# mx-mark/VideoTransformer-pytorch

Measured on AMD Instinct MI355X. Metric: clips/sec TimeSformer-B divided_space_time 8x3x224x224 fwd+bwd (whole job), higher is better.
Workload: dtype bf16

## Files before the change

### videotransformer-pytorch_amd/csrc/api.hip

```cpp
#include <limits.h>
#include <stdarg.h>
#include <stdlib.h>
#include <string.h>
#include <string>
#include <vector>
#include "common.h"

namespace vtx {

static thread_local char g_err[512] = "";

void set_error(const char* fmt, ...) {
  va_list ap;
  va_start(ap, fmt);
  vsnprintf(g_err, sizeof(g_err), fmt, ap);
  va_end(ap);
}

int check_launch(const char* what) {
  hipError_t e = hipGetLastError();
  if (e != hipSuccess) {
    set_error("%s: launch failed: %s", what, hipGetErrorString(e));
    return VTX_ELAUNCH;
  }
  return VTX_OK;
}

static const char* const kNtNames[] = {"auto", "pp256", "dma2", "ring128x3", "ring128x4k32", "ring256x3", "ring256x3k32", "ring256x4k32"};
static const char* const kAttnF32Names[] = {"valu", "mfma"};
static const char* const kTnNames[] = {"auto", "pp256", "ring", "dma2", "w4"};

enum OptKind { OPT_FLAG, OPT_INT, OPT_CLAMP, OPT_ENUM, OPT_ADDR };
struct OptRow { const char* id[2]; OptKind kind; int Options::*field; int lo, hi, mult; const char* const* names; };
#define VTX_ENUM(names) 0, (int)(sizeof(names) / sizeof(*names)) - 1, 1, names
static const OptRow kOptions[] = {
    {{"VTX_GEMM_NT", "gemm_nt"}, OPT_ENUM, &Options::gemm_nt, VTX_ENUM(kNtNames)},
    {{"VTX_GEMM_TN", "gemm_tn"}, OPT_ENUM, &Options::gemm_tn, VTX_ENUM(kTnNames)},
    {{"VTX_GEMM_NODMA", "gemm_nodma"}, OPT_FLAG, &Options::gemm_nodma},
    {{"VTX_TN_SAFE", "tn_safe"}, OPT_FLAG, &Options::tn_safe},
    {{"VTX_TN_CUS", "tn_cus"}, OPT_INT, &Options::tn_cus, 32, 1024, 1},
    {{"VTX_ATTN_VALU", "attn_valu"}, OPT_FLAG, &Options::attn_valu},
    {{"VTX_ATTN_LONG", "attn_long"}, OPT_FLAG, &Options::attn_long},
    {{"VTX_ATTN_F32", "attn_f32"}, OPT_ENUM, &Options::attn_f32, VTX_ENUM(kAttnF32Names)},
    {{"VTX_ATTN_HD", "attn_hd"}, OPT_ENUM, &Options::attn_hd, VTX_ENUM(kAttnF32Names)},
    {{"VTX_ATTN_HW_FWD", "attn_hw_fwd"}, OPT_INT, &Options::attn_hw_fwd, 0, INT_MAX, 1},
    {{"VTX_ATTN_HW_BWD", "attn_hw_bwd"}, OPT_INT, &Options::attn_hw_bwd, 0, INT_MAX, 1},
    {{"VTX_ATTN_FUSED", "attn_fused"}, OPT_CLAMP, &Options::attn_fused, 0, 2},
    {{"VTX_ATTN_FWD_STREAM", "attn_fwd_stream"}, OPT_FLAG, &Options::attn_fwd_stream},
    {{"VTX_ATTN_DKV", "attn_dkv"}, OPT_INT, &Options::attn_dkv, 0, 4, 1},
    {{"VTX_GEMM_PP_GRID", "pp_grid"}, OPT_INT, &Options::pp_grid, 8, 4096, 8},
    {{"VTX_GEMM_PP_CG", "pp_cg"}, OPT_INT, &Options::pp_cg, 0, INT_MAX, 1},
    {{"VTX_GEMM_PP_EPI", "pp_epi"}, OPT_INT, &Options::pp_epi, INT_MIN, INT_MAX, 1},
    {{"VTX_GEMM_PP_CONT", "pp_cont"}, OPT_FLAG, &Options::pp_cont},
// ... 161 lines not shown
```

### videotransformer-pytorch_amd/csrc/common.h

```cpp
#pragma once
#include <hip/hip_runtime.h>
#include <stdint.h>
#include <atomic>
#include <stdio.h>
#include "../../include/vtx.h"

namespace vtx {

typedef __attribute__((ext_vector_type(8))) __bf16 bf16x8;
typedef __attribute__((ext_vector_type(4))) __bf16 bf16x4;
typedef __attribute__((ext_vector_type(4))) float f32x4;
typedef __attribute__((ext_vector_type(4))) unsigned int u32x4;
typedef __attribute__((ext_vector_type(16))) float f32x16;
typedef __attribute__((ext_vector_type(4))) short s16x4;
typedef unsigned short bf16raw;

__host__ __device__ inline float bf2f(bf16raw v) {
  union { uint32_t u; float f; } c; c.u = ((uint32_t)v) << 16; return c.f;
}
__host__ __device__ inline bf16raw f2bf(float f) {
#if defined(__HIP_DEVICE_COMPILE__)
  union { __bf16 b; bf16raw r; } c; c.b = (__bf16)f; return c.r;
#else
  union { uint32_t u; float f; } c; c.f = f;
// ... 97 lines not shown
#pragma clang fp contract(off)
  float cdf, g;
  gelu_parts(x, cdf, g);
  return x * cdf;
}
__device__ inline float gelu_erf_grad(float x) {
#pragma clang fp contract(off)
  float cdf, g;
  gelu_parts(x, cdf, g);
  const float xs = x * 0.3989422804014327f;
  return fmaf(xs, g, cdf);
}
__device__ inline void gelu_erf_both(float x, float& val, float& grad) {
#pragma clang fp contract(off)
  float cdf, g;
  gelu_parts(x, cdf, g);
  const float xs = x * 0.3989422804014327f;
  grad = fmaf(xs, g, cdf);
  val = x * cdf;
}

enum { NT_AUTO = 0, NT_PP256, NT_DMA2, NT_RING128X3, NT_RING128X4K32, NT_RING256X3, NT_RING256X3K32, NT_RING256X4K32,
       NT_REG, NT_F32 };
enum { TN_AUTO = 0, TN_PP256, TN_RING, TN_DMA2, TN_W4 };
struct Options {
  int gemm_nt = NT_AUTO;
  int gemm_tn = TN_AUTO;
  int gemm_nodma = 0;
  int tn_safe = 0;
  int tn_cus = 256;
  int attn_valu = 0;
  int attn_long = 1;
  int attn_f32 = 1;
  int attn_hw_fwd = 16;
  int attn_hw_bwd = 4;
  int attn_fused = 2;
  int attn_fwd_stream = 1;
  int attn_dkv = 3;
  int ln_rows = 3;
  int pp_grid = 256;
  int pp_cg = 0;
  int pp_epi = 0;
  int pp_cont = 1;
  unsigned long long pp_trace = 0;
  int attn_hd = 1;
};
Options& options();
// ... 48 lines not shown
```

### videotransformer-pytorch_amd/csrc/gemm_tn.hip

```cpp
#include <stdlib.h>
#include <string>
#include "gemm_common.h"

namespace vtx {

struct TnOut {
  float* slab; long slab_stride;
  int N1, N2;
  float* cslab;
  int cs_fold;
};

struct TnTile { int split, t1, t2, r0, c0, m_begin, m_end; };
template <int TM, int TC, bool REMAINDER, typename Id>
__device__ __forceinline__ TnTile tn_tile_of(Id bid, int M, int m_per_split, int tiles2, int tiles12) {
  TnTile t;
  t.split = bid / tiles12;
  const int tile = bid - t.split * tiles12;
  t.t1 = tile / tiles2; t.t2 = tile - t.t1 * tiles2;
  t.r0 = t.t1 * TM; t.c0 = t.t2 * TC;
  t.m_begin = t.split * m_per_split;
  if (REMAINDER) t.m_end = (t.split == (int)(gridDim.x / tiles12) - 1) ? M : t.m_begin + m_per_split;
  else t.m_end = min(M, t.m_begin + m_per_split);
  return t;
}
template <int TM, int TC, bool REMAP, bool REMAINDER>
__device__ __forceinline__ TnTile tn_tile(int M, int m_per_split, int tiles2, int tiles12) {
  if (REMAP) return tn_tile_of<TM, TC, REMAINDER>(xcd_remap(blockIdx.x, gridDim.x), M, m_per_split, tiles2, tiles12);
  return tn_tile_of<TM, TC, REMAINDER>((unsigned)blockIdx.x, M, m_per_split, tiles2, tiles12);
}

template <int NI, int NJ>
__device__ __forceinline__ void tn_zero(f32x16 (&acc)[NI][NJ]) {
#pragma unroll
  for (int i = 0; i < NI; ++i)
#pragma unroll
    for (int j = 0; j < NJ; ++j)
#pragma unroll
      for (int r = 0; r < 16; ++r) acc[i][j][r] = 0.f;
}

__device__ __forceinline__ void tn_cs_add(float (&cs)[8], const u32x4& v) {
#pragma unroll
  for (int j = 0; j < 4; ++j) {
    cs[2 * j] += __uint_as_float(v[j] << 16);
    cs[2 * j + 1] += __uint_as_float(v[j] & 0xffff0000u);
  }
}
template <int TC, int NV>
__device__ __forceinline__ void tn_cs_put(float* red, int row_lane, int col, const float (&cs)[NV]) {
#pragma unroll
  for (int j = 0; j < NV; ++j) red[row_lane * TC + col + j] = cs[j];
}
template <int RL, int TC>
__device__ __forceinline__ void tn_cs_fold(const float* red, const TnOut& o, const TnTile& t, int copy, int tid) {
  __syncthreads();
  if (tid < TC && t.r0 + tid < o.N1) {
    float a = 0.f;
#pragma unroll
    for (int r = 0; r < RL; ++r) a += red[r * TC + tid];
    o.cslab[(long)t.split * o.slab_stride + (long)copy * o.N1 + t.r0 + tid] = a;
  }
  __syncthreads();
// ... 14 lines not shown
  }
}

template <int LD>
__device__ __forceinline__ bf16x8 tn_tr_pair(const bf16raw* p) {
  union { bf16x8 v; s16x4 h[2]; } u;
  u.h[0] = __builtin_amdgcn_ds_read_tr16_b64_v4i16((s16x4 __attribute__((address_space(3)))*)(p));
  u.h[1] = __builtin_amdgcn_ds_read_tr16_b64_v4i16((s16x4 __attribute__((address_space(3)))*)(p + 4 * LD));
  return u.v;
}
typedef __attribute__((address_space(3))) char tn_lds_char;
template <int OFF> __device__ inline s16x4 tn_tr_read(unsigned addr) {
  s16x4 d;
  asm volatile("ds_read_b64_tr_b16 %0, %1 offset:%2" : "=v"(d) : "v"(addr), "n"(OFF) : "memory");
  return d;
}
template <int OFF, int ROW4>
__device__ __forceinline__ bf16x8 tn_tr_frag(unsigned addr) {
  union { bf16x8 v; s16x4 h[2]; } u;
  u.h[0] = tn_tr_read<OFF>(addr);
  u.h[1] = tn_tr_read<OFF + ROW4>(addr);
  return u.v;
}

template <int ROWS, int CHUNKS, int THREADS>
__device__ __forceinline__ void tn_stage_ragged(bf16raw* dst, const bf16raw* __restrict__ src, long ld, const vtx_rowmap& map,
                                                int mt, int m_end, int col0, int ncols, int tid) {
  constexpr int RPP = THREADS / CHUNKS;
#pragma unroll
  for (int it = 0; it < ROWS / RPP; ++it) {
    const int row = tid / CHUNKS + RPP * it;
    const int lc = (tid % CHUNKS) ^ ((row & 3) << 2);
    uint4 v = make_uint4(0, 0, 0, 0);
    if (mt + row < m_end && col0 + lc * 8 < ncols)
      v = *reinterpret_cast<const uint4*>(src + map_row(map, mt + row) * ld + col0 + lc * 8);
    *reinterpret_cast<uint4*>(dst + row * (8 * CHUNKS) + (tid % CHUNKS) * 8) = v;
  }
}

constexpr int TN_BKM = 64;
constexpr int TN_LD = 160;
constexpr int TN_BKM32 = 16;
constexpr int TN_LD32 = 128;

template <bool SAFE>
__global__ __launch_bounds__(NT_THREADS) void gemm_tn_bf16_kernel(
// ... 389 lines not shown
    tn_cs_put<256>(red, cs_row, cs_chunk * 8, csum);
    tn_cs_fold<16, 256>(red, out, t, t2, tid);
  }
  float* stg = reinterpret_cast<float*>(smem) + wave * 32 * STAGE_LD;
#pragma unroll
  for (int mi = 0; mi < 2; ++mi) {
    stage_acc_half(stg, acc[mi], lane);
    __builtin_amdgcn_s_waitcnt(0xc07f);
    __builtin_amdgcn_wave_barrier();
    tn_store<4, STAGE_LD, 1>(out, stg, t.split, r0 + wm * 64 + mi * 32, c0 + wn * 64 + (lane & 7) * 8, lane);
    __builtin_amdgcn_s_waitcnt(0xc07f);
    __builtin_amdgcn_wave_barrier();
  }
}

constexpr int TP_BK = 64, TP_THREADS = 512;
constexpr int TP_REGION = TP_BK * 128;
constexpr int TP_BUF = 4 * TP_REGION;
constexpr int TP_RING_BYTES = 2 * TP_BUF * 2;
constexpr int TP_STG_LD = 64;
constexpr int TP_LDS_BYTES = TP_RING_BYTES + 8 * 16 * TP_STG_LD * 4;

constexpr int TP_FAR = 1 << 28;
template <int PPW>
struct TnFeeder {
  bf16raw* lds;
  int wave, lane, last_valid;
  long lda, ldb;
  int grp_a, grp_b;
  int prow0, rc, acol_l;
  unsigned voff_a, voff_b;
  int trm[4], crs[4], vld[4];
  const char* sp[4];
  long step64_a, step64_b;
  long skipb_a, skipb_b;

  __device__ __forceinline__ TnFeeder(bf16raw* lds_, int wave_, int lane_, const bf16raw* A, long lda_, const vtx_rowmap& amap,
                                      const bf16raw* B, long ldb_, const vtx_rowmap& bmap, int M, const TnTile& t, int last_valid_)
      : lds(lds_), wave(wave_), lane(lane_), last_valid(last_valid_), lda(lda_), ldb(ldb_), grp_a(amap.grp), grp_b(bmap.grp) {
    const int pc0 = wave * PPW, sub = pc0 >> 3;
    prow0 = (pc0 & 7) * 8 + (lane >> 3);
    rc = sub * 64 + ((lane & 7) ^ (((prow0 >> 1) & 1) << 2)) * 8;
    acol_l = (rc >> 6) * 128 + (rc & 63);
    voff_a = 2u * (unsigned)(prow0 * (int)lda + acol_l); voff_b = 2u * (unsigned)(prow0 * (int)ldb + rc);
    step64_a = 2L * TP_BK * lda; step64_b = 2L * TP_BK * ldb;
    skipb_a = 2L * amap.skip * lda; skipb_b = 2L * bmap.skip * ldb;
#pragma unroll
    for (int k = 0; k < 4; ++k) {
      const bool isA = k == 0 || k == 3;
      const vtx_rowmap& mp = isA ? amap : bmap;
      const int g = mp.grp;
      const int q = g > 0 ? t.m_begin / g : 0;
      trm[k] = g > 0 ? t.m_begin - q * g : 0;
      crs[k] = g > 0 ? g - trm[k] : TP_FAR;
      vld[k] = M - t.m_begin;
      const long phys0 = (long)mp.base + t.m_begin + (long)q * mp.skip;
      sp[k] = reinterpret_cast<const char*>(isA ? A + phys0 * lda + t.r0 + (k == 3 ? 64 : 0) : B + phys0 * ldb + t.c0 + (k == 2 ? 128 : 0));
    }
  }
  __device__ __forceinline__ bf16raw* piece(int kind, int kt, int j) const {
    return lds + (kt & 1) * TP_BUF + kind * TP_REGION + wave * (PPW * 512) + j * 512;
  }
  __device__ __forceinline__ void issue_piece(int kind, int kt, int j) {
    bf16raw* dst = piece(kind, kt, j);
    const bool isA = kind == 0 || kind == 3;
    const char* lo = sp[kind];
    const char* hi = lo + (isA ? skipb_a : skipb_b);
    const unsigned vo = isA ? voff_a : voff_b, vc = 2u * (unsigned)(isA ? acol_l : rc);
    const unsigned step8 = 16u * (unsigned)(isA ? lda : ldb);
    const int row = prow0 + 8 * j;
    if (crs[kind] >= TP_BK && vld[kind] >= TP_BK) {
      const unsigned m0v = (unsigned)(unsigned long)(tn_lds_char*)dst;
      asm volatile("s_mov_b32 m0, %2\n\ts_nop 0\n\tglobal_load_lds_dwordx4 %0, %1"
                   :: "v"(vo + j * step8), "s"(lo), "s"(m0v) : "memory", "m0");
      return;
    }
    const char* base = row >= crs[kind] ? hi : lo;
    const unsigned o = row < vld[kind] ? vo + j * step8 : vc;
    dma16(reinterpret_cast<const bf16raw*>(base + o), dst);
  }
  __device__ __forceinline__ void issue(int kind, int kt) {
#pragma unroll
    for (int j = 0; j < PPW; ++j) issue_piece(kind, kt, j);
  }
  __device__ __forceinline__ void advance(int kind) {
    const bool isA = kind == 0 || kind == 3;
    const int g = isA ? grp_a : grp_b;
    sp[kind] += isA ? step64_a : step64_b;
    vld[kind] -= TP_BK;
    if (g > 0) {
      trm[kind] += TP_BK;
      if (trm[kind] >= g) { trm[kind] -= g; sp[kind] += isA ? skipb_a : skipb_b; }
      crs[kind] = g - trm[kind];
    }
  }
  __device__ __forceinline__ void zero_tail(int kt) {
#pragma unroll
    for (int kind = 0; kind < 4; ++kind)
#pragma unroll
      for (int j = 0; j < PPW; ++j)
        if (prow0 + 8 * j >= last_valid) *reinterpret_cast<uint4*>(piece(kind, kt, j) + lane * 8) = make_uint4(0, 0, 0, 0);
  }
};

template <int R>
struct TnCsLane {
  unsigned sub, row, pc;
  __device__ __forceinline__ explicit TnCsLane(unsigned tid) : sub(tid / (8 * R)), row((tid >> 3) & (R - 1)), pc(tid & 7) {}
  __device__ __forceinline__ unsigned lds_off() const { return sub * 4096 + row * 64 + pc * 8; }
  __device__ __forceinline__ int tile_col() const { return sub * 128 + (pc ^ (((row >> 1) & 1) << 2)) * 8; }
};

template <int HALF>
__device__ __forceinline__ void tn_epi16(const TnOut& o, float* stg, const f32x16& a0, const f32x16& a1, int split, int r_base, int c, int lane) {
  const int col = lane & 31, rhalf = (lane >> 5) * 4;
#pragma unroll
  for (int r = 0; r < 8; ++r) stg[((r & 3) + 8 * (r >> 2) + rhalf) * TP_STG_LD + col] = a0[8 * HALF + r];
#pragma unroll
  for (int r = 0; r < 8; ++r) stg[((r & 3) + 8 * (r >> 2) + rhalf) * TP_STG_LD + 32 + col] = a1[8 * HALF + r];
  lgkm0();
  __builtin_amdgcn_wave_barrier();
  tn_store<2, TP_STG_LD, 2>(o, stg, split, r_base, c, lane);
  lgkm0();
  __builtin_amdgcn_wave_barrier();
}

template <bool TRACE>
__global__ __launch_bounds__(TP_THREADS, 2) void gemm_tn_bf16_pp_kernel(
    int M, int m_per_split, const bf16raw* __restrict__ A, long lda, vtx_rowmap amap,
    const bf16raw* __restrict__ B, long ldb, vtx_rowmap bmap, int tiles2, int tiles12, TnOut out, long long* __restrict__ trace) {
  extern __shared__ __attribute__((aligned(16))) char smem[];
  bf16raw* lds = reinterpret_cast<bf16raw*>(smem);
  const int tid = threadIdx.x, lane = tid & 63;
  const int wave = __builtin_amdgcn_readfirstlane(tid >> 6);
  const int wr = wave >> 2, wc = wave & 3;
  int trace_kt = -1;
  auto stamp = [&](int e) {
    if constexpr (TRACE) {
      if (tid == 0 && trace_kt >= 0)
        trace[((long)blockIdx.x * 8 + trace_kt) * 24 + e] = (long long)__builtin_amdgcn_s_memtime();
    }
  };
  const TnTile t = tn_tile<256, 256, true, true>(M, m_per_split, tiles2, tiles12);
  const int t2 = t.t2, r0 = t.r0, c0 = t.c0;
  const int span = t.m_end - t.m_begin;
  const int nk = (span + TP_BK - 1) / TP_BK;
  const int last_valid = span - (nk - 1) * TP_BK;
  TnFeeder<2> fd(lds, wave, lane, A, lda, amap, B, ldb, bmap, M, t, last_valid);

  f32x16 acc[4][2];
  tn_zero(acc);

  const int tr_row = 8 * (lane >> 5) + ((lane & 15) >> 2);
  const int tr_sw = ((lane >> 3) & 1) << 2;
  const int cl = 16 * ((lane >> 4) & 1) + 4 * (lane & 3);
  int fa_off[2], fb_off;
#pragma unroll
  for (int i = 0; i < 2; ++i) {
    const int cc = i * 32 + cl;
    fa_off[i] = wr * 4096 + tr_row * 64 + (((cc >> 3) ^ tr_sw) << 3) + (cc & 7);
  }
  {
    const int cc = (wc & 1) * 32 + cl;
    fb_off = (wc >> 1) * 4096 + tr_row * 64 + (((cc >> 3) ^ tr_sw) << 3) + (cc & 7);
  }
  const unsigned lds_b = (unsigned)(unsigned long)(tn_lds_char*)smem;
  const unsigned fa_addr[2] = {lds_b + 2u * fa_off[0], lds_b + 2u * fa_off[1]}, fb_addr = lds_b + 2u * fb_off;
  const bool want_cs = out.cslab != nullptr;
  bool do_cs = false;
  int cs_next = t2;
  float cs0[8] = {0, 0, 0, 0, 0, 0, 0, 0}, cs1[8] = {0, 0, 0, 0, 0, 0, 0, 0};
#define TP_COLSUM(buf_, kind_, cs_)                                                                      \
  if (do_cs) {                                                                                           \
    u32x4 v_[2];                                                                                         \
                                 \
    unsigned t_ = threadIdx.x;                                                                           \
    asm volatile("" : "+v"(t_));                                                                         \
    const unsigned ca_ = lds_b + 2u * ((t_ >> 8) * 4096 + ((t_ >> 3) & 31) * 64 + (t_ & 7) * 8);        \
    asm volatile("ds_read_b128 %0, %2\n\tds_read_b128 %1, %2 offset:4096\n\ts_waitcnt lgkmcnt(0)"        \
                 : "=&v"(v_[0]), "=&v"(v_[1]) : "v"(ca_ + 2u * ((buf_) * TP_BUF + (kind_) * TP_REGION)) : "memory"); \
    tn_cs_add(cs_, v_[0]);                                                                               \
    tn_cs_add(cs_, v_[1]);                                                                               \
  }
#define TP_READ_A(buf_, kind_)                                                                           \
  _Pragma("unroll") for (int i = 0; i < 2; ++i) {                                                        \
    const unsigned a_ = fa_addr[i] + 2u * ((buf_) * TP_BUF + (kind_) * TP_REGION);                       \
    fa[i][0] = tn_tr_frag<0, 512>(a_);    fa[i][1] = tn_tr_frag<2048, 512>(a_);                          \
    fa[i][2] = tn_tr_frag<4096, 512>(a_); fa[i][3] = tn_tr_frag<6144, 512>(a_);                          \
  }
#define TP_READ_B_Q(buf_, kind_, fb_, Q_)                                                                \
  fb_[Q_] = tn_tr_frag<(Q_) * 2048, 512>(fb_addr + 2u * ((buf_) * TP_BUF + (kind_) * TP_REGION))
#define TP_READ_B(buf_, kind_, fb_)                                                                      \
  { TP_READ_B_Q(buf_, kind_, fb_, 0); TP_READ_B_Q(buf_, kind_, fb_, 1); TP_READ_B_Q(buf_, kind_, fb_, 2); TP_READ_B_Q(buf_, kind_, fb_, 3); }
#define TP_PIN_A() asm volatile("" : "+v"(fa[0][0]), "+v"(fa[0][1]), "+v"(fa[0][2]), "+v"(fa[0][3]),      \
                                     "+v"(fa[1][0]), "+v"(fa[1][1]), "+v"(fa[1][2]), "+v"(fa[1][3]))
#define TP_PIN_B(fb_) asm volatile("" : "+v"(fb_[0]), "+v"(fb_[1]), "+v"(fb_[2]), "+v"(fb_[3]))
#define TP_MFMA1(i_, ks_, i0_, j_, fb_)                                                                  \
  acc[(i0_) + (i_)][j_] = __builtin_amdgcn_mfma_f32_32x32x16_bf16(fa[i_][ks_], fb_[ks_], acc[(i0_) + (i_)][j_], 0, 0, 0); \
  __builtin_amdgcn_sched_barrier(0);
#ifndef VTX_TP_PRIO
#define VTX_TP_PRIO 0
#endif
#define TP_PRIO_ON() do { if (VTX_TP_PRIO == 1) __builtin_amdgcn_s_setprio(1); else if (VTX_TP_PRIO == 3) __builtin_amdgcn_s_setprio(0); } while (0)
#define TP_PRIO_OFF() do { if (VTX_TP_PRIO == 1) __builtin_amdgcn_s_setprio(0); else if (VTX_TP_PRIO == 3) __builtin_amdgcn_s_setprio(1); } while (0)
#define TP_MMA(i0_, j_, fb_, H0_, H1_, H2_, H3_, H4_, H5_)                                               \
  TP_PRIO_ON();                                                                                          \
  __builtin_amdgcn_sched_barrier(0);                                                                     \
  TP_MFMA1(0, 0, i0_, j_, fb_) H0_; __builtin_amdgcn_sched_barrier(0);                                   \
  TP_MFMA1(1, 0, i0_, j_, fb_) H1_; __builtin_amdgcn_sched_barrier(0);                                   \
  TP_MFMA1(0, 1, i0_, j_, fb_) H2_; __builtin_amdgcn_sched_barrier(0);                                   \
  TP_MFMA1(1, 1, i0_, j_, fb_) H3_; __builtin_amdgcn_sched_barrier(0);                                   \
  TP_MFMA1(0, 2, i0_, j_, fb_) H4_; __builtin_amdgcn_sched_barrier(0);                                   \
  TP_MFMA1(1, 2, i0_, j_, fb_) H5_; __builtin_amdgcn_sched_barrier(0);                                   \
  TP_MFMA1(0, 3, i0_, j_, fb_)                                                                           \
  TP_MFMA1(1, 3, i0_, j_, fb_)                                                                           \
  TP_PRIO_OFF();
#define TP_BAR() __builtin_amdgcn_s_barrier()

  bf16x8 fa[2][4], fb0[4], fb1[4];
  fd.issue(0, 0); fd.advance(0); fd.issue(1, 0); fd.advance(1); fd.issue(2, 0); fd.advance(2); fd.issue(3, 0); fd.advance(3);
  fd.issue(0, 1); fd.advance(0); fd.issue(1, 1); fd.advance(1); fd.issue(2, 1); fd.advance(2);
  wait_vmcnt<8>();
  TP_BAR();
  if (wr == 1) TP_BAR();
  if (VTX_TP_PRIO == 2 && wr == 1) __builtin_amdgcn_s_setprio(1);
  if (VTX_TP_PRIO == 3) __builtin_amdgcn_s_setprio(1);
#define TP_KTILE(kt_, X_, Y_)                                                                            \
  {                                                                                                      \
    const int kt = (kt_);                                                                                \
    const int buf = kt & 1;                                                                              \
    const bool n1 = kt + 1 < nk, n2 = kt + 2 < nk;                                                       \
    do_cs = want_cs && kt == cs_next;                                                                    \
    if (do_cs) cs_next += tiles2;                                                                        \
    if constexpr (TRACE) trace_kt = (kt >= 8 && kt < 16) ? kt - 8 : -1;                                  \
    stamp(0);                                                                                            \
     \
    if (kt >= 1 && n1) fd.advance(2);                 \
    TP_READ_A(buf, 0);                                                                                   \
    TP_COLSUM(buf, 0, cs0);                                                                              \
    lgkm0();                                                                                             \
    stamp(1);                                                                                            \
    stamp(2);                                                                                            \
// ... 43 lines not shown
      wait_vmcnt<6>();                                                              \
    }                                                                                                    \
    stamp(12);                                                                                           \
    TP_BAR();                                                                                            \
    stamp(13);                                                                                           \
    TP_MMA(2, 0, X_, if (n2) fd.issue_piece(2, kt + 2, 0), if (n2) fd.issue_piece(2, kt + 2, 1),         \
           if (n1) TP_READ_B_Q(buf ^ 1, 1, Y_, 0), if (n1) TP_READ_B_Q(buf ^ 1, 1, Y_, 1),               \
           if (n1) TP_READ_B_Q(buf ^ 1, 1, Y_, 2), if (n1) TP_READ_B_Q(buf ^ 1, 1, Y_, 3));              \
    stamp(18);                                                                                           \
    TP_BAR();                                                                                            \
    stamp(14);                                                                                           \
  }
  TP_READ_B(0, 1, fb0);
  for (int kt2 = 0; kt2 < nk; kt2 += 2) {
    TP_KTILE(kt2, fb0, fb1)
    if (kt2 + 1 < nk) TP_KTILE(kt2 + 1, fb1, fb0)
  }
#undef TP_KTILE
  if (wr == 0) TP_BAR();
  if (VTX_TP_PRIO >= 2) __builtin_amdgcn_s_setprio(0);
#undef TP_COLSUM
#undef TP_READ_B_Q
#undef TP_MFMA1
#undef TP_PIN_A
#undef TP_PIN_B
#undef TP_READ_A
#undef TP_READ_B
#undef TP_MMA
#undef TP_BAR
  if (want_cs) {
    float* red = reinterpret_cast<float*>(smem);
    const TnCsLane<32> csl(tid);
    tn_cs_put<256>(red, csl.row, csl.tile_col(), cs0);
    tn_cs_put<256>(red, csl.row, csl.tile_col() + 64, cs1);
    tn_cs_fold<32, 256>(red, out, t, t2, tid);
  }
  float* stg = reinterpret_cast<float*>(smem + TP_RING_BYTES) + wave * 16 * TP_STG_LD;
  const int c = c0 + ((lane & 7) >> 2) * 128 + wc * 32 + (lane & 3) * 8;
#pragma unroll
  for (int mi = 0; mi < 4; ++mi) {
    tn_epi16<0>(out, stg, acc[mi][0], acc[mi][1], t.split, r0 + wr * 128 + mi * 32, c, lane);
    tn_epi16<1>(out, stg, acc[mi][0], acc[mi][1], t.split, r0 + wr * 128 + mi * 32 + 16, c, lane);
  }
}

constexpr int TW_THREADS = 256;
constexpr int TW_LDS_BYTES = TP_RING_BYTES + 4 * 16 * TP_STG_LD * 4;

template <bool WANT_CS>
__global__ __launch_bounds__(TW_THREADS, 1) void gemm_tn_bf16_w4_kernel(
    int M, int m_per_split, const bf16raw* __restrict__ A, long lda, vtx_rowmap amap,
    const bf16raw* __restrict__ B, long ldb, vtx_rowmap bmap, int tiles2, int tiles12, TnOut out) {
  extern __shared__ __attribute__((aligned(16))) char smem[];
  bf16raw* lds = reinterpret_cast<bf16raw*>(smem);
  const int tid = threadIdx.x, lane = tid & 63;
  const int wave = __builtin_amdgcn_readfirstlane(tid >> 6);
  const int wr = wave >> 1, wc = wave & 1;
  const TnTile t = tn_tile<256, 256, true, true>(M, m_per_split, tiles2, tiles12);
  const int t2 = t.t2, r0 = t.r0, c0 = t.c0;
  const int span = t.m_end - t.m_begin;
  const int nk = (span + TP_BK - 1) / TP_BK;
  const int last_valid = span - (nk - 1) * TP_BK;
  TnFeeder<4> fd(lds, wave, lane, A, lda, amap, B, ldb, bmap, M, t, last_valid);

  f32x16 acc[4][4];
// ... 171 lines not shown
  float* stg = reinterpret_cast<float*>(smem + TP_RING_BYTES) + wave * 16 * TP_STG_LD;
#pragma unroll
  for (int jp = 0; jp < 2; ++jp)
#pragma unroll
    for (int mi = 0; mi < 4; ++mi) {
      const int r = r0 + wr * 128 + mi * 32, c = c0 + jp * 128 + wc * 64 + (lane_e & 7) * 8;
      __builtin_amdgcn_sched_barrier(0);
      tn_epi16<0>(out, stg, acc[mi][2 * jp], acc[mi][2 * jp + 1], t.split, r, c, lane_e);
      __builtin_amdgcn_sched_barrier(0);
      tn_epi16<1>(out, stg, acc[mi][2 * jp], acc[mi][2 * jp + 1], t.split, r + 16, c, lane_e);
      __builtin_amdgcn_sched_barrier(0);
    }
}

static int tp_splits(int M, int N1, int N2) {
  const int tiles = cdiv(N1, 256) * cdiv(N2, 256);
  int s = options().tn_cus / tiles;
  const int max_s = M / 128;
  if (s > max_s) s = max_s;
  return s < 1 ? 1 : s;
}
static bool tp_eligible(int M, int N1, int N2) { return M >= 4096 && N1 % 256 == 0 && N2 % 256 == 0; }
static bool tp_map_ok(const vtx_rowmap& m) { return m.grp == 0 || m.grp > TP_BK; }

template <typename T>
__global__ __launch_bounds__(256) void colsum_kernel(int M, int N, int rows_per_blk, const T* __restrict__ A,
                                                     long lda, vtx_rowmap amap, float* __restrict__ part) {
  __shared__ float red[8][256 + 8];
  const int cc = threadIdx.x & 31, rl = threadIdx.x >> 5;
  const int n = blockIdx.x * 256 + cc * 8;
  const long m0 = (long)blockIdx.y * rows_per_blk;
  const long m1 = min((long)M, m0 + rows_per_blk);
  float acc[8] = {0, 0, 0, 0, 0, 0, 0, 0};
  if (n < N) {
    for (long m = m0 + rl; m < m1; m += 8) {
      float v[8];
      load8(A + map_row(amap, m) * lda + n, v);
#pragma unroll
      for (int j = 0; j < 8; ++j) acc[j] += v[j];
    }
  }
#pragma unroll
  for (int j = 0; j < 8; ++j) red[rl][cc * 8 + j] = acc[j];
  __syncthreads();
  const int c = threadIdx.x;
  const int ncol = blockIdx.x * 256 + c;
  if (ncol < N) {
    float a = 0.f;
#pragma unroll
    for (int r = 0; r < 8; ++r) a += red[r][c];
    part[(long)blockIdx.y * N + ncol] = a;
  }
}

static int tn_splits(int M, int N1, int N2) {
  const int tiles = cdiv(N1, 128) * cdiv(N2, 128);
  int s = cdiv(768, tiles);
  const int max_s = M / 256 > 0 ? M / 256 : 1;
  if (s > max_s) s = max_s;
  if (s < 1) s = 1;
  return s;
}
static int colsum_blocks(int M) {
  int b = cdiv(M, 256);
  return b > 256 ? 256 : (b < 1 ? 1 : b);
}

enum TnKernel { TK_F32, TK_SAFE, TK_NODMA, TK_DMA2, TK_RING, TK_PP256, TK_PP256_TRACE, TK_W4 };
struct TnPlan {
  TnKernel kernel;
  unsigned grid, block;
  size_t lds;
  int tiles2, tiles12;
  int slabs, m_per;
  int cs_fold;
  long slab_stride;
  long red_n; int red_fold;
};

static size_t tn_slab_bytes(int slabs, long slab_stride) { return (size_t)slabs * (size_t)slab_stride * sizeof(float); }
static int tn_ws_slabs(int M, int N1, int N2) {
  const int s = tn_splits(M, N1, N2), s_p = tp_eligible(M, N1, N2) ? tp_splits(M, N1, N2) : 0;
  return s_p > s ? s_p : s;
}

static TnPlan tn_plan(int dtype, int M, int N1, int N2, const vtx_rowmap& amap, const vtx_rowmap& bmap, bool has_colsum,
                      const Options& o) {
  TnPlan p;
  const int tiles2 = cdiv(N2, 128);
  auto small = [&](TnKernel k, int tile_m, size_t need) {
    p.kernel = k; p.block = NT_THREADS; p.lds = STAGE_BYTES > need ? STAGE_BYTES : need;
    p.tiles2 = tiles2; p.tiles12 = cdiv(N1, 128) * tiles2; p.cs_fold = 1;
    p.slabs = tn_splits(M, N1, N2);
    p.m_per = cdiv(cdiv(M, p.slabs), tile_m) * tile_m;
  };
  const bool pp_fits = tp_eligible(M, N1, N2) && tp_map_ok(amap) && tp_map_ok(bmap);
  if (dtype != VTX_BF16) {
    small(TK_F32, TN_BKM32, (size_t)2 * TN_BKM32 * TN_LD32 * 4);
  } else if (o.tn_safe || o.gemm_nodma) {
    small(o.tn_safe ? TK_SAFE : TK_NODMA, TN_BKM, (size_t)2 * TN_BKM * TN_LD * 2);
  } else if (pp_fits && (o.gemm_tn == TN_W4 || o.gemm_tn == TN_PP256 || o.gemm_tn == TN_AUTO)) {
    static_assert(TP_BK == 64, "tp_splits caps the slab count at M / 128 = M / (2 * TP_BK)");
    const bool w4 = o.gemm_tn == TN_W4;
    p.kernel = w4 ? TK_W4 : o.pp_trace ? TK_PP256_TRACE : TK_PP256;
    p.block = w4 ? TW_THREADS : TP_THREADS; p.lds = w4 ? TW_LDS_BYTES : TP_LDS_BYTES;
    p.tiles2 = cdiv(N2, 256); p.tiles12 = cdiv(N1, 256) * p.tiles2; p.cs_fold = p.tiles2;
    p.slabs = tp_splits(M, N1, N2);
    p.m_per = (M / p.slabs) / TP_BK * TP_BK;
  } else if (o.gemm_tn != TN_DMA2 && M >= 1024) {
    const size_t ring_bytes = (size_t)TR_NBUF * TR_STAGE * 2, stage_bytes = (size_t)8 * 32 * STAGE_LD * 4;
    p.kernel = TK_RING; p.block = 512; p.lds = ring_bytes > stage_bytes ? ring_bytes : stage_bytes;
    p.tiles2 = tiles2; p.tiles12 = cdiv(N1, 256) * tiles2; p.cs_fold = tiles2;
    int s = 512 / p.tiles12;
    if (s > tn_ws_slabs(M, N1, N2)) s = tn_ws_slabs(M, N1, N2);
    if (s > M / (2 * TR_BKM)) s = M / (2 * TR_BKM);
    p.slabs = s < 1 ? 1 : s;
    p.m_per = cdiv(cdiv(M, p.slabs), TR_BKM) * TR_BKM;
  } else {
    small(TK_DMA2, TN_BKM, (size_t)4 * TN_BKM * TN_DLD * 2);
  }
  p.grid = (unsigned)(p.tiles12 * p.slabs);
  p.slab_stride = (long)N1 * N2 + (long)p.cs_fold * N1;
  p.red_n = (long)N1 * N2 + (has_colsum ? N1 : 0);
  p.red_fold = has_colsum ? p.cs_fold : 1;
  return p;
}

// ... 19 lines not shown
  VTX_REQUIRE(d->A && d->B && d->C && d->workspace, VTX_EINVAL, "gemm_tn: null pointer");
  VTX_REQUIRE(d->ldc == d->N2, VTX_EINVAL, "gemm_tn: C must be contiguous (ldc == N2)");
  VTX_REQUIRE(closed_form(d->amap) && closed_form(d->bmap), VTX_EINVAL, "gemm_tn: row maps must be in closed form (no table)");
  VTX_REQUIRE(d->dtype == VTX_F32 || d->dtype == VTX_BF16, VTX_EINVAL, "gemm_tn: bad dtype");
  const long vec = d->dtype == VTX_BF16 ? 8 : 4;
  VTX_REQUIRE(aligned16(d->A) && aligned16(d->B) && aligned16(d->C) && aligned16(d->workspace) &&
                  d->lda % vec == 0 && d->ldb % vec == 0, VTX_EALIGN, "gemm_tn: 16-byte alignment required");
  VTX_REQUIRE(d->ws_bytes >= vtx_gemm_tn_workspace(d->M, d->N1, d->N2), VTX_EWS, "gemm_tn: workspace too small");

  const TnPlan p = tn_plan(d->dtype, d->M, d->N1, d->N2, d->amap, d->bmap, d->colsum != nullptr, options());
  VTX_REQUIRE(tn_slab_bytes(p.slabs, p.slab_stride) <= d->ws_bytes, VTX_EWS, "gemm_tn: the plan's %d slabs of %ld floats outgrow the workspace",
              p.slabs, p.slab_stride);
  const long w_elems = (long)d->N1 * d->N2;
  TnOut out;
  out.slab = (float*)d->workspace; out.slab_stride = p.slab_stride; out.N1 = d->N1; out.N2 = d->N2;
  out.cslab = d->colsum ? out.slab + w_elems : nullptr; out.cs_fold = p.cs_fold;
  hipStream_t st = as_stream(stream);
  switch (p.kernel) {
    case TK_F32: tn_launch<gemm_tn_f32_kernel, float>(p, d, out, st); break;
    case TK_SAFE: tn_launch<gemm_tn_bf16_kernel<true>, bf16raw>(p, d, out, st); break;
    case TK_NODMA: tn_launch<gemm_tn_bf16_kernel<false>, bf16raw>(p, d, out, st); break;
    case TK_DMA2: tn_launch<gemm_tn_bf16_dma_kernel, bf16raw>(p, d, out, st); break;
    case TK_RING: tn_launch<gemm_tn_bf16_ring_kernel, bf16raw>(p, d, out, st); break;
    case TK_PP256: tn_launch<gemm_tn_bf16_pp_kernel<false>, bf16raw>(p, d, out, st, (long long*)nullptr); break;
    case TK_PP256_TRACE: tn_launch<gemm_tn_bf16_pp_kernel<true>, bf16raw>(p, d, out, st, reinterpret_cast<long long*>(options().pp_trace)); break;
    case TK_W4:
      if (out.cslab) tn_launch<gemm_tn_bf16_w4_kernel<true>, bf16raw>(p, d, out, st);
      else tn_launch<gemm_tn_bf16_w4_kernel<false>, bf16raw>(p, d, out, st);
      break;
  }
  const int rc = check_launch("gemm_tn");
  if (rc) return rc;
  return launch_reduce_partials(out.slab, p.slabs, p.slab_stride, p.red_n, d->C, d->accumulate, 1.0f, st,
                                d->colsum, w_elems, d->colsum_accumulate, p.red_fold, d->N1);
}

extern "C" size_t vtx_colsum_workspace(int M, int N) {
  return (size_t)colsum_blocks(M) * (size_t)N * sizeof(float);
}

extern "C" int vtx_colsum(int dtype, int M, int N, const void* A, long lda, vtx_rowmap amap, float* out,
                          int accumulate, void* workspace, size_t ws_bytes, void* stream) {
  VTX_REQUIRE(M > 0 && N > 0 && N % 8 == 0, VTX_EINVAL, "colsum: bad shape M=%d N=%d", M, N);
  VTX_REQUIRE(A && out && workspace, VTX_EINVAL, "colsum: null pointer");
  VTX_REQUIRE(ws_bytes >= vtx_colsum_workspace(M, N), VTX_EWS, "colsum: workspace too small");
  const long vec = dtype == VTX_BF16 ? 8 : 4;
  VTX_REQUIRE(aligned16(A) && lda % vec == 0, VTX_EALIGN, "colsum: 16-byte alignment required");
  const int nb = colsum_blocks(M);
// ... 14 lines not shown
```

Before: 775.0.

## Switch TN weight-gradient GEMM to 16x16x32 MFMA with row-bit-3 LDS swizzle

The pp256 TN GEMM kernel, which computes the weight gradients, gets a variant that uses 16x16x32 bf16 MFMA instructions instead of 32x32x16. It changes the fragment layout and per-lane LDS addressing, and adds an extra XOR swizzle on row bit 3 in the feeder, tail zeroing and column-sum lanes. The auto path now selects this variant by default, and the old 32x32 path stays reachable through a new option. The aim is better MFMA issue and fewer LDS bank conflicts. In exchange there are more MFMA instructions per tile and a riskier swizzle scheme.

```diff
diff --git a/videotransformer-pytorch_amd/csrc/api.hip b/videotransformer-pytorch_amd/csrc/api.hip
--- a/videotransformer-pytorch_amd/csrc/api.hip
+++ b/videotransformer-pytorch_amd/csrc/api.hip
@@ -28,7 +28,7 @@
 
 static const char* const kNtNames[] = {"auto", "pp256", "dma2", "ring128x3", "ring128x4k32", "ring256x3", "ring256x3k32", "ring256x4k32"};
 static const char* const kAttnF32Names[] = {"valu", "mfma"};
-static const char* const kTnNames[] = {"auto", "pp256", "ring", "dma2", "w4"};
+static const char* const kTnNames[] = {"auto", "pp256", "ring", "dma2", "w4", "pp256_mfma32", "pp256_mfma16"};
 
 enum OptKind { OPT_FLAG, OPT_INT, OPT_CLAMP, OPT_ENUM, OPT_ADDR };
 struct OptRow { const char* id[2]; OptKind kind; int Options::*field; int lo, hi, mult; const char* const* names; };
diff --git a/videotransformer-pytorch_amd/csrc/common.h b/videotransformer-pytorch_amd/csrc/common.h
--- a/videotransformer-pytorch_amd/csrc/common.h
+++ b/videotransformer-pytorch_amd/csrc/common.h
@@ -143,7 +143,7 @@
 
 enum { NT_AUTO = 0, NT_PP256, NT_DMA2, NT_RING128X3, NT_RING128X4K32, NT_RING256X3, NT_RING256X3K32, NT_RING256X4K32,
        NT_REG, NT_F32 };
-enum { TN_AUTO = 0, TN_PP256, TN_RING, TN_DMA2, TN_W4 };
+enum { TN_AUTO = 0, TN_PP256, TN_RING, TN_DMA2, TN_W4, TN_PP256_M32, TN_PP256_M16 };
 struct Options {
   int gemm_nt = NT_AUTO;
   int gemm_tn = TN_AUTO;
diff --git a/videotransformer-pytorch_amd/csrc/gemm_tn.hip b/videotransformer-pytorch_amd/csrc/gemm_tn.hip
--- a/videotransformer-pytorch_amd/csrc/gemm_tn.hip
+++ b/videotransformer-pytorch_amd/csrc/gemm_tn.hip
@@ -1,5 +1,6 @@
 #include <stdlib.h>
 #include <string>
+#include <type_traits>
 #include "gemm_common.h"
 
 namespace vtx {
@@ -39,6 +40,15 @@
 #pragma unroll
       for (int r = 0; r < 16; ++r) acc[i][j][r] = 0.f;
 }
+template <int NI, int NJ>
+__device__ __forceinline__ void tn_zero(f32x4 (&acc)[NI][NJ]) {
+#pragma unroll
+  for (int i = 0; i < NI; ++i)
+#pragma unroll
+    for (int j = 0; j < NJ; ++j)
+#pragma unroll
+      for (int r = 0; r < 4; ++r) acc[i][j][r] = 0.f;
+}
 
 __device__ __forceinline__ void tn_cs_add(float (&cs)[8], const u32x4& v) {
 #pragma unroll
@@ -99,6 +109,9 @@
   u.h[1] = tn_tr_read<OFF + ROW4>(addr);
   return u.v;
 }
+
+template <int OFF>
+__device__ __forceinline__ bf16x8 tn_tr_frag4(unsigned addr) { return tn_tr_frag<OFF, 512>(addr); }
 
 template <int ROWS, int CHUNKS, int THREADS>
 __device__ __forceinline__ void tn_stage_ragged(bf16raw* dst, const bf16raw* __restrict__ src, long ld, const vtx_rowmap& map,
@@ -534,14 +547,16 @@
 constexpr int TP_LDS_BYTES = TP_RING_BYTES + 8 * 16 * TP_STG_LD * 4;
 
 constexpr int TP_FAR = 1 << 28;
-template <int PPW>
+template <int PPW, bool SW3 = false>
 struct TnFeeder {
+  static_assert(!SW3 || PPW == 2, "the row-bit-3 image is written for two pieces per wave: piece 0 even, piece 1 odd");
   bf16raw* lds;
   int wave, lane, last_valid;
   long lda, ldb;
   int grp_a, grp_b;
   int prow0, rc, acol_l;
   unsigned voff_a, voff_b;
+  unsigned voff_a2, voff_b2;
   int trm[4], crs[4], vld[4];
   const char* sp[4];
   long step64_a, step64_b;
@@ -555,6 +570,9 @@
     rc = sub * 64 + ((lane & 7) ^ (((prow0 >> 1) & 1) << 2)) * 8;
     acol_l = (rc >> 6) * 128 + (rc & 63);
     voff_a = 2u * (unsigned)(prow0 * (int)lda + acol_l); voff_b = 2u * (unsigned)(prow0 * (int)ldb + rc);
+    if constexpr (SW3) {
+      voff_a2 = 2u * (unsigned)((prow0 + 8) * (int)lda + (acol_l ^ 16)); voff_b2 = 2u * (unsigned)((prow0 + 8) * (int)ldb + (rc ^ 16));
+    }
     step64_a = 2L * TP_BK * lda; step64_b = 2L * TP_BK * ldb;
     skipb_a = 2L * amap.skip * lda; skipb_b = 2L * bmap.skip * ldb;
 #pragma unroll
@@ -578,8 +596,10 @@
     const bool isA = kind == 0 || kind == 3;
     const char* lo = sp[kind];
     const char* hi = lo + (isA ? skipb_a : skipb_b);
-    const unsigned vo = isA ? voff_a : voff_b, vc = 2u * (unsigned)(isA ? acol_l : rc);
     const unsigned step8 = 16u * (unsigned)(isA ? lda : ldb);
+    const bool odd = SW3 && (j & 1);
+    const unsigned vo = odd ? (isA ? voff_a2 : voff_b2) - step8 : isA ? voff_a : voff_b;
+    const unsigned vc = (2u * (unsigned)(isA ? acol_l : rc)) ^ (odd ? 32u : 0u);
     const int row = prow0 + 8 * j;
     if (crs[kind] >= TP_BK && vld[kind] >= TP_BK) {
       const unsigned m0v = (unsigned)(unsigned long)(tn_lds_char*)dst;
@@ -607,6 +627,18 @@
     }
   }
   __device__ __forceinline__ void zero_tail(int kt) {
+    if constexpr (SW3) {
+      unsigned t_ = threadIdx.x, z_ = 0;
+      asm volatile("" : "+v"(t_), "+v"(z_));
+      const unsigned l_ = t_ & 63;
+#pragma unroll
+      for (int kind = 0; kind < 4; ++kind)
+#pragma unroll
+        for (int j = 0; j < PPW; ++j)
+          if ((int)(((wave * PPW) & 7) * 8 + (l_ >> 3)) + 8 * j >= last_valid)
+            *reinterpret_cast<uint4*>(piece(kind, kt, j) + l_ * 8) = make_uint4(z_, z_, z_, z_);
+      return;
+    }
 #pragma unroll
     for (int kind = 0; kind < 4; ++kind)
 #pragma unroll
@@ -615,12 +647,15 @@
   }
 };
 
-template <int R>
+template <int R, bool SW3 = false>
 struct TnCsLane {
+  static_assert(!SW3 || R == 32, "the rows of a thread must share bit 3 as well");
   unsigned sub, row, pc;
   __device__ __forceinline__ explicit TnCsLane(unsigned tid) : sub(tid / (8 * R)), row((tid >> 3) & (R - 1)), pc(tid & 7) {}
   __device__ __forceinline__ unsigned lds_off() const { return sub * 4096 + row * 64 + pc * 8; }
-  __device__ __forceinline__ int tile_col() const { return sub * 128 + (pc ^ (((row >> 1) & 1) << 2)) * 8; }
+  __device__ __forceinline__ int tile_col() const {
+    return sub * 128 + (pc ^ (((row >> 1) & 1) << 2) ^ (SW3 ? ((row >> 3) & 1) << 1 : 0u)) * 8;
+  }
 };
 
 template <int HALF>
@@ -637,7 +672,20 @@
   __builtin_amdgcn_wave_barrier();
 }
 
-template <bool TRACE>
+__device__ __forceinline__ void tn_epi16_mf16(const TnOut& o, float* stg, const f32x4 (&a)[4], int split, int r_base, int c, int lane) {
+  const int col = lane & 15, row = 4 * (lane >> 4);
+#pragma unroll
+  for (int jb = 0; jb < 4; ++jb)
+#pragma unroll
+    for (int r = 0; r < 4; ++r) stg[(row + r) * TP_STG_LD + 16 * jb + col] = a[jb][r];
+  lgkm0();
+  __builtin_amdgcn_wave_barrier();
+  tn_store<2, TP_STG_LD, 2>(o, stg, split, r_base, c, lane);
+  lgkm0();
+  __builtin_amdgcn_wave_barrier();
+}
+
+template <bool TRACE, bool MF16>
 __global__ __launch_bounds__(TP_THREADS, 2) void gemm_tn_bf16_pp_kernel(
     int M, int m_per_split, const bf16raw* __restrict__ A, long lda, vtx_rowmap amap,
     const bf16raw* __restrict__ B, long ldb, vtx_rowmap bmap, int tiles2, int tiles12, TnOut out, long long* __restrict__ trace) {
@@ -649,8 +697,11 @@
   int trace_kt = -1;
   auto stamp = [&](int e) {
     if constexpr (TRACE) {
-      if (tid == 0 && trace_kt >= 0)
-        trace[((long)blockIdx.x * 8 + trace_kt) * 24 + e] = (long long)__builtin_amdgcn_s_memtime();
+      if (tid == 0 && trace_kt >= 0) {
+        long long* slot = trace + ((long)blockIdx.x * 8 + trace_kt) * 24;
+        slot[e] = (long long)__builtin_amdgcn_s_memtime();
+        if (e == 0 || e == 14) slot[e == 0 ? 19 : 20] = (long long)__builtin_amdgcn_s_memrealtime();
+      }
     }
   };
   const TnTile t = tn_tile<256, 256, true, true>(M, m_per_split, tiles2, tiles12);
@@ -658,26 +709,27 @@
   const int span = t.m_end - t.m_begin;
   const int nk = (span + TP_BK - 1) / TP_BK;
   const int last_valid = span - (nk - 1) * TP_BK;
-  TnFeeder<2> fd(lds, wave, lane, A, lda, amap, B, ldb, bmap, M, t, last_valid);
-
-  f32x16 acc[4][2];
+  TnFeeder<2, MF16> fd(lds, wave, lane, A, lda, amap, B, ldb, bmap, M, t, last_valid);
+
+  std::conditional_t<MF16, f32x4[8][4], f32x16[4][2]> acc;
   tn_zero(acc);
 
-  const int tr_row = 8 * (lane >> 5) + ((lane & 15) >> 2);
-  const int tr_sw = ((lane >> 3) & 1) << 2;
-  const int cl = 16 * ((lane >> 4) & 1) + 4 * (lane & 3);
-  int fa_off[2], fb_off;
-#pragma unroll
-  for (int i = 0; i < 2; ++i) {
-    const int cc = i * 32 + cl;
-    fa_off[i] = wr * 4096 + tr_row * 64 + (((cc >> 3) ^ tr_sw) << 3) + (cc & 7);
-  }
-  {
-    const int cc = (wc & 1) * 32 + cl;
-    fb_off = (wc >> 1) * 4096 + tr_row * 64 + (((cc >> 3) ^ tr_sw) << 3) + (cc & 7);
-  }
+  constexpr int NFA = MF16 ? 4 : 2, NFB = MF16 ? 2 : 1, CW = MF16 ? 16 : 32;
+  const int tr_row = 8 * (MF16 ? lane >> 4 : lane >> 5) + ((lane & 15) >> 2);
+  const int tr_sw = (((lane >> 3) & 1) << 2) ^ (MF16 ? ((lane >> 4) & 1) << 1 : 0);
+  const int cl = (MF16 ? 0 : 16 * ((lane >> 4) & 1)) + 4 * (lane & 3);
   const unsigned lds_b = (unsigned)(unsigned long)(tn_lds_char*)smem;
-  const unsigned fa_addr[2] = {lds_b + 2u * fa_off[0], lds_b + 2u * fa_off[1]}, fb_addr = lds_b + 2u * fb_off;
+  unsigned fa_addr[NFA], fb_addr[NFB];
+#pragma unroll
+  for (int i = 0; i < NFA; ++i) {
+    const int cc = i * CW + cl;
+    fa_addr[i] = lds_b + 2u * (wr * 4096 + tr_row * 64 + (((cc >> 3) ^ tr_sw) << 3) + (cc & 7));
+  }
+#pragma unroll
+  for (int i = 0; i < NFB; ++i) {
+    const int cc = (wc & 1) * 32 + i * CW + cl;
+    fb_addr[i] = lds_b + 2u * ((wc >> 1) * 4096 + tr_row * 64 + (((cc >> 3) ^ tr_sw) << 3) + (cc & 7));
+  }
   const bool want_cs = out.cslab != nullptr;
   bool do_cs = false;
   int cs_next = t2;
@@ -695,21 +747,58 @@
     tn_cs_add(cs_, v_[1]);                                                                               \
   }
 #define TP_READ_A(buf_, kind_)                                                                           \
-  _Pragma("unroll") for (int i = 0; i < 2; ++i) {                                                        \
+  _Pragma("unroll") for (int i = 0; i < NFA; ++i) {                                                      \
     const unsigned a_ = fa_addr[i] + 2u * ((buf_) * TP_BUF + (kind_) * TP_REGION);                       \
-    fa[i][0] = tn_tr_frag<0, 512>(a_);    fa[i][1] = tn_tr_frag<2048, 512>(a_);                          \
-    fa[i][2] = tn_tr_frag<4096, 512>(a_); fa[i][3] = tn_tr_frag<6144, 512>(a_);                          \
+    if constexpr (MF16) {                                                                                \
+      fa[2 * i] = tn_tr_frag4<0>(a_); fa[2 * i + 1] = tn_tr_frag4<4096>(a_);                             \
+    } else {                                                                                             \
+      fa[4 * i] = tn_tr_frag4<0>(a_);        fa[4 * i + 1] = tn_tr_frag4<2048>(a_);                      \
+      fa[4 * i + 2] = tn_tr_frag4<4096>(a_); fa[4 * i + 3] = tn_tr_frag4<6144>(a_);                      \
+    }                                                                                                    \
   }
 #define TP_READ_B_Q(buf_, kind_, fb_, Q_)                                                                \
-  fb_[Q_] = tn_tr_frag<(Q_) * 2048, 512>(fb_addr + 2u * ((buf_) * TP_BUF + (kind_) * TP_REGION))
+  {                                                                                                      \
+    const unsigned b_ = fb_addr[(Q_) & (NFB - 1)] + 2u * ((buf_) * TP_BUF + (kind_) * TP_REGION);        \
+    if constexpr (MF16) fb_[Q_] = tn_tr_frag4<((Q_) >> 1) * 4096>(b_); else fb_[Q_] = tn_tr_frag4<(Q_) * 2048>(b_); \
+  }
 #define TP_READ_B(buf_, kind_, fb_)                                                                      \
   { TP_READ_B_Q(buf_, kind_, fb_, 0); TP_READ_B_Q(buf_, kind_, fb_, 1); TP_READ_B_Q(buf_, kind_, fb_, 2); TP_READ_B_Q(buf_, kind_, fb_, 3); }
-#define TP_PIN_A() asm volatile("" : "+v"(fa[0][0]), "+v"(fa[0][1]), "+v"(fa[0][2]), "+v"(fa[0][3]),      \
-                                     "+v"(fa[1][0]), "+v"(fa[1][1]), "+v"(fa[1][2]), "+v"(fa[1][3]))
+#define TP_PIN_A() asm volatile("" : "+v"(fa[0]), "+v"(fa[1]), "+v"(fa[2]), "+v"(fa[3]), "+v"(fa[4]), "+v"(fa[5]), "+v"(fa[6]), "+v"(fa[7]))
 #define TP_PIN_B(fb_) asm volatile("" : "+v"(fb_[0]), "+v"(fb_[1]), "+v"(fb_[2]), "+v"(fb_[3]))
 #define TP_MFMA1(i_, ks_, i0_, j_, fb_)                                                                  \
-  acc[(i0_) + (i_)][j_] = __builtin_amdgcn_mfma_f32_32x32x16_bf16(fa[i_][ks_], fb_[ks_], acc[(i0_) + (i_)][j_], 0, 0, 0); \
+  acc[(i0_) + (i_)][j_] = __builtin_amdgcn_mfma_f32_32x32x16_bf16(fa[4 * (i_) + (ks_)], fb_[ks_], acc[(i0_) + (i_)][j_], 0, 0, 0); \
   __builtin_amdgcn_sched_barrier(0);
+#define TP_MFMA16(m_, i0_, j_, fb_)                                                                      \
+  acc[2 * (i0_) + (((m_) >> 1) & 3)][2 * (j_) + ((m_) & 1)] = __builtin_amdgcn_mfma_f32_16x16x32_bf16(   \
+      fa[2 * (((m_) >> 1) & 3) + ((m_) >> 3)], fb_[2 * ((m_) >> 3) + ((m_) & 1)], acc[2 * (i0_) + (((m_) >> 1) & 3)][2 * (j_) + ((m_) & 1)], 0, 0, 0); \
+  __builtin_amdgcn_sched_barrier(0);
+#define TP_MMA16_SLOTS(i0_, j_, fb_, S0_, S1_, S2_, S3_, S4_, S5_, S6_, S7_, S8_, S9_, S10_, S11_, S12_, S13_, S14_) \
+  TP_MFMA16(0, i0_, j_, fb_) S0_; __builtin_amdgcn_sched_barrier(0);                                     \
+  TP_MFMA16(1, i0_, j_, fb_) S1_; __builtin_amdgcn_sched_barrier(0);                                     \
+  TP_MFMA16(2, i0_, j_, fb_) S2_; __builtin_amdgcn_sched_barrier(0);                                     \
+  TP_MFMA16(3, i0_, j_, fb_) S3_; __builtin_amdgcn_sched_barrier(0);                                     \
+  TP_MFMA16(4, i0_, j_, fb_) S4_; __builtin_amdgcn_sched_barrier(0);                                     \
+  TP_MFMA16(5, i0_, j_, fb_) S5_; __builtin_amdgcn_sched_barrier(0);                                     \
+  TP_MFMA16(6, i0_, j_, fb_) S6_; __builtin_amdgcn_sched_barrier(0);                                     \
+  TP_MFMA16(7, i0_, j_, fb_) S7_; __builtin_amdgcn_sched_barrier(0);                                     \
+  TP_MFMA16(8, i0_, j_, fb_) S8_; __builtin_amdgcn_sched_barrier(0);                                     \
+  TP_MFMA16(9, i0_, j_, fb_) S9_; __builtin_amdgcn_sched_barrier(0);                                     \
+  TP_MFMA16(10, i0_, j_, fb_) S10_; __builtin_amdgcn_sched_barrier(0);                                   \
+  TP_MFMA16(11, i0_, j_, fb_) S11_; __builtin_amdgcn_sched_barrier(0);                                   \
+  TP_MFMA16(12, i0_, j_, fb_) S12_; __builtin_amdgcn_sched_barrier(0);                                   \
+  TP_MFMA16(13, i0_, j_, fb_) S13_; __builtin_amdgcn_sched_barrier(0);                                   \
+  TP_MFMA16(14, i0_, j_, fb_) S14_; __builtin_amdgcn_sched_barrier(0);                                   \
+  TP_MFMA16(15, i0_, j_, fb_)
+#ifndef VTX_TP_HOOKS
+#define VTX_TP_HOOKS 0
+#endif
+#if VTX_TP_HOOKS == 0
+#define TP_MMA16(i0_, j_, fb_, H0_, H1_, H2_, H3_, H4_, H5_) TP_MMA16_SLOTS(i0_, j_, fb_, H0_, , H1_, , H2_, , H3_, , H4_, , H5_, , , , )
+#elif VTX_TP_HOOKS == 1
+#define TP_MMA16(i0_, j_, fb_, H0_, H1_, H2_, H3_, H4_, H5_) TP_MMA16_SLOTS(i0_, j_, fb_, H0_, H1_, H2_, H3_, H4_, H5_, , , , , , , , , )
+#else
+#define TP_MMA16(i0_, j_, fb_, H0_, H1_, H2_, H3_, H4_, H5_) TP_MMA16_SLOTS(i0_, j_, fb_, H0_, , , H1_, , , H2_, , , H3_, , , H4_, , H5_)
+#endif
 #ifndef VTX_TP_PRIO
 #define VTX_TP_PRIO 0
 #endif
@@ -718,18 +807,22 @@
 #define TP_MMA(i0_, j_, fb_, H0_, H1_, H2_, H3_, H4_, H5_)                                               \
   TP_PRIO_ON();                                                                                          \
   __builtin_amdgcn_sched_barrier(0);                                                                     \
-  TP_MFMA1(0, 0, i0_, j_, fb_) H0_; __builtin_amdgcn_sched_barrier(0);                                   \
-  TP_MFMA1(1, 0, i0_, j_, fb_) H1_; __builtin_amdgcn_sched_barrier(0);                                   \
-  TP_MFMA1(0, 1, i0_, j_, fb_) H2_; __builtin_amdgcn_sched_barrier(0);                                   \
-  TP_MFMA1(1, 1, i0_, j_, fb_) H3_; __builtin_amdgcn_sched_barrier(0);                                   \
-  TP_MFMA1(0, 2, i0_, j_, fb_) H4_; __builtin_amdgcn_sched_barrier(0);                                   \
-  TP_MFMA1(1, 2, i0_, j_, fb_) H5_; __builtin_amdgcn_sched_barrier(0);                                   \
-  TP_MFMA1(0, 3, i0_, j_, fb_)                                                                           \
-  TP_MFMA1(1, 3, i0_, j_, fb_)                                                                           \
+  if constexpr (MF16) {                                                                                  \
+    TP_MMA16(i0_, j_, fb_, H0_, H1_, H2_, H3_, H4_, H5_)                                                 \
+  } else {                                                                                               \
+    TP_MFMA1(0, 0, i0_, j_, fb_) H0_; __builtin_amdgcn_sched_barrier(0);                                 \
+    TP_MFMA1(1, 0, i0_, j_, fb_) H1_; __builtin_amdgcn_sched_barrier(0);                                 \
+    TP_MFMA1(0, 1, i0_, j_, fb_) H2_; __builtin_amdgcn_sched_barrier(0);                                 \
+    TP_MFMA1(1, 1, i0_, j_, fb_) H3_; __builtin_amdgcn_sched_barrier(0);                                 \
+    TP_MFMA1(0, 2, i0_, j_, fb_) H4_; __builtin_amdgcn_sched_barrier(0);                                 \
+    TP_MFMA1(1, 2, i0_, j_, fb_) H5_; __builtin_amdgcn_sched_barrier(0);                                 \
+    TP_MFMA1(0, 3, i0_, j_, fb_)                                                                         \
+    TP_MFMA1(1, 3, i0_, j_, fb_)                                                                         \
+  }                                                                                                      \
   TP_PRIO_OFF();
 #define TP_BAR() __builtin_amdgcn_s_barrier()
 
-  bf16x8 fa[2][4], fb0[4], fb1[4];
+  bf16x8 fa[8], fb0[4], fb1[4];
   fd.issue(0, 0); fd.advance(0); fd.issue(1, 0); fd.advance(1); fd.issue(2, 0); fd.advance(2); fd.issue(3, 0); fd.advance(3);
   fd.issue(0, 1); fd.advance(0); fd.issue(1, 1); fd.advance(1); fd.issue(2, 1); fd.advance(2);
   wait_vmcnt<8>();
@@ -819,6 +912,9 @@
 #undef TP_COLSUM
 #undef TP_READ_B_Q
 #undef TP_MFMA1
+#undef TP_MFMA16
+#undef TP_MMA16
+#undef TP_MMA16_SLOTS
 #undef TP_PIN_A
 #undef TP_PIN_B
 #undef TP_READ_A
@@ -827,17 +923,22 @@
 #undef TP_BAR
   if (want_cs) {
     float* red = reinterpret_cast<float*>(smem);
-    const TnCsLane<32> csl(tid);
+    const TnCsLane<32, MF16> csl(tid);
     tn_cs_put<256>(red, csl.row, csl.tile_col(), cs0);
     tn_cs_put<256>(red, csl.row, csl.tile_col() + 64, cs1);
     tn_cs_fold<32, 256>(red, out, t, t2, tid);
   }
   float* stg = reinterpret_cast<float*>(smem + TP_RING_BYTES) + wave * 16 * TP_STG_LD;
   const int c = c0 + ((lane & 7) >> 2) * 128 + wc * 32 + (lane & 3) * 8;
-#pragma unroll
-  for (int mi = 0; mi < 4; ++mi) {
-    tn_epi16<0>(out, stg, acc[mi][0], acc[mi][1], t.split, r0 + wr * 128 + mi * 32, c, lane);
-    tn_epi16<1>(out, stg, acc[mi][0], acc[mi][1], t.split, r0 + wr * 128 + mi * 32 + 16, c, lane);
+  if constexpr (MF16) {
+#pragma unroll
+    for (int bi = 0; bi < 8; ++bi) tn_epi16_mf16(out, stg, acc[bi], t.split, r0 + wr * 128 + bi * 16, c, lane);
+  } else {
+#pragma unroll
+    for (int mi = 0; mi < 4; ++mi) {
+      tn_epi16<0>(out, stg, acc[mi][0], acc[mi][1], t.split, r0 + wr * 128 + mi * 32, c, lane);
+      tn_epi16<1>(out, stg, acc[mi][0], acc[mi][1], t.split, r0 + wr * 128 + mi * 32 + 16, c, lane);
+    }
   }
 }
 
@@ -1055,6 +1156,7 @@
 }
 static bool tp_eligible(int M, int N1, int N2) { return M >= 4096 && N1 % 256 == 0 && N2 % 256 == 0; }
 static bool tp_map_ok(const vtx_rowmap& m) { return m.grp == 0 || m.grp > TP_BK; }
+static bool tp_mf16(int M, int N1, int N2) { (void)M; (void)N1; (void)N2; return true; }
 
 template <typename T>
 __global__ __launch_bounds__(256) void colsum_kernel(int M, int N, int rows_per_blk, const T* __restrict__ A,
@@ -1099,7 +1201,7 @@
   return b > 256 ? 256 : (b < 1 ? 1 : b);
 }
 
-enum TnKernel { TK_F32, TK_SAFE, TK_NODMA, TK_DMA2, TK_RING, TK_PP256, TK_PP256_TRACE, TK_W4 };
+enum TnKernel { TK_F32, TK_SAFE, TK_NODMA, TK_DMA2, TK_RING, TK_PP256, TK_PP256_TRACE, TK_W4, TK_PP256_M32, TK_PP256_M32_TRACE };
 struct TnPlan {
   TnKernel kernel;
   unsigned grid, block;
@@ -1132,10 +1234,12 @@
     small(TK_F32, TN_BKM32, (size_t)2 * TN_BKM32 * TN_LD32 * 4);
   } else if (o.tn_safe || o.gemm_nodma) {
     small(o.tn_safe ? TK_SAFE : TK_NODMA, TN_BKM, (size_t)2 * TN_BKM * TN_LD * 2);
-  } else if (pp_fits && (o.gemm_tn == TN_W4 || o.gemm_tn == TN_PP256 || o.gemm_tn == TN_AUTO)) {
+  } else if (pp_fits && (o.gemm_tn == TN_W4 || o.gemm_tn == TN_PP256 || o.gemm_tn == TN_AUTO || o.gemm_tn == TN_PP256_M32 || o.gemm_tn == TN_PP256_M16)) {
     static_assert(TP_BK == 64, "tp_splits caps the slab count at M / 128 = M / (2 * TP_BK)");
     const bool w4 = o.gemm_tn == TN_W4;
-    p.kernel = w4 ? TK_W4 : o.pp_trace ? TK_PP256_TRACE : TK_PP256;
+    const bool m32 = o.gemm_tn == TN_PP256_M32 || (o.gemm_tn != TN_PP256_M16 && !tp_mf16(M, N1, N2));
+    p.kernel = w4 ? TK_W4 : m32 ? (o.pp_trace ? TK_PP256_M32_TRACE : TK_PP256_M32)
+                                : o.pp_trace ? TK_PP256_TRACE : TK_PP256;
     p.block = w4 ? TW_THREADS : TP_THREADS; p.lds = w4 ? TW_LDS_BYTES : TP_LDS_BYTES;
     p.tiles2 = cdiv(N2, 256); p.tiles12 = cdiv(N1, 256) * p.tiles2; p.cs_fold = p.tiles2;
     p.slabs = tp_splits(M, N1, N2);
@@ -1201,8 +1305,10 @@
     case TK_NODMA: tn_launch<gemm_tn_bf16_kernel<false>, bf16raw>(p, d, out, st); break;
     case TK_DMA2: tn_launch<gemm_tn_bf16_dma_kernel, bf16raw>(p, d, out, st); break;
     case TK_RING: tn_launch<gemm_tn_bf16_ring_kernel, bf16raw>(p, d, out, st); break;
-    case TK_PP256: tn_launch<gemm_tn_bf16_pp_kernel<false>, bf16raw>(p, d, out, st, (long long*)nullptr); break;
-    case TK_PP256_TRACE: tn_launch<gemm_tn_bf16_pp_kernel<true>, bf16raw>(p, d, out, st, reinterpret_cast<long long*>(options().pp_trace)); break;
+    case TK_PP256: tn_launch<gemm_tn_bf16_pp_kernel<false, true>, bf16raw>(p, d, out, st, (long long*)nullptr); break;
+    case TK_PP256_TRACE: tn_launch<gemm_tn_bf16_pp_kernel<true, true>, bf16raw>(p, d, out, st, reinterpret_cast<long long*>(options().pp_trace)); break;
+    case TK_PP256_M32: tn_launch<gemm_tn_bf16_pp_kernel<false, false>, bf16raw>(p, d, out, st, (long long*)nullptr); break;
+    case TK_PP256_M32_TRACE: tn_launch<gemm_tn_bf16_pp_kernel<true, false>, bf16raw>(p, d, out, st, reinterpret_cast<long long*>(options().pp_trace)); break;
     case TK_W4:
       if (out.cslab) tn_launch<gemm_tn_bf16_w4_kernel<true>, bf16raw>(p, d, out, st);
       else tn_launch<gemm_tn_bf16_w4_kernel<false>, bf16raw>(p, d, out, st);
```

Measured after the change: 779.2, median of 6. Within noise of the previous version (+0.5%).
